# nghorbani/moshpp

Hardware: NVIDIA H100
Metric: mocap frames solved/sec (Stage-II) (higher is better)
Workload: dtype f32

## Files before the change

moshpp_b200/csrc/mosh2.cu:

```cuda
#include "../../include/mosh2.h"

#include <cuda_runtime.h>

#include <cstdarg>
#include <cstdio>
#include <cstdlib>
#include <algorithm>
#include <cstring>
#include <map>
#include <mutex>
#include <new>
#include <string>
#include <vector>

#include "mesh_distance.cuh"
#include "mosh2_device.cuh"
#include "mosh2_host.h"

namespace {

thread_local std::string g_err;

int fail(int code, const char *fmt, ...) {
    char buf[512];
// ... 270 lines not shown
    int *d_status = nullptr, *d_counters = nullptr, *d_totals = nullptr;
    long long *d_prof = nullptr;
    void *h_obs = nullptr, *h_out = nullptr;
    uint8_t *h_vis = nullptr;
    void *d_lin = nullptr;
    size_t lin_bytes = 0;
    int lin_mode = 0, lin_step = 1;
    mosh2_host::LinLayout lin{};
    struct RangeSlot { void *h = nullptr, *d = nullptr; size_t bytes = 0; cudaEvent_t done = nullptr; };
    std::vector<RangeSlot> range_slots;
    int *h_status = nullptr, *h_counters = nullptr;
    std::vector<mosh2_model *> models;
    std::vector<unsigned char> h_models;
    void *d_models = nullptr;
    int *d_model_of_chunk = nullptr;
    size_t n_obs = 0, n_out = 0;
    size_t o_fullpose = 0, o_pose = 0, o_trans = 0, o_dmpls = 0, o_mk = 0, o_errs = 0;
};

namespace {

template <class real, bool BIG>
cudaError_t launch_kernel(mosh2_job *j, const mosh2::Model<real> &m, const mosh2::Job<real> &job, int threads) {
    const mosh2_host::Layout<real, BIG> L = mosh2_host::layout<real, BIG>(m, mosh2::kSmemHeader, threads);
    const cudaError_t e = cudaFuncSetAttribute(mosh2_stageii_kernel<real, BIG>, cudaFuncAttributeMaxDynamicSharedMemorySize, int(j->smem));
    if (e != cudaSuccess) return e;
    mosh2_stageii_kernel<real, BIG><<<j->launch_blocks, threads, j->smem, j->stream>>>(m, job, L.w, L.d);
    return cudaGetLastError();
}

template <class real, bool BIG>
cudaError_t launch_multi_kernel(mosh2_job *j, const mosh2::Job<real> &job, int threads) {
    const mosh2::Model<real> &m = *reinterpret_cast<const mosh2::Model<real> *>(j->h_models.data());
    const mosh2_host::Layout<real, BIG> L = mosh2_host::layout<real, BIG>(m, mosh2_host::multi_smem_header<real>(), threads);
    const cudaError_t e = cudaFuncSetAttribute(mosh2_stageii_multi_kernel<real, BIG>, cudaFuncAttributeMaxDynamicSharedMemorySize, int(j->smem));
    if (e != cudaSuccess) return e;
    mosh2_stageii_multi_kernel<real, BIG><<<j->launch_blocks, threads, j->smem, j->stream>>>(
        static_cast<const mosh2::Model<real> *>(j->d_models), j->d_model_of_chunk, job, L.w, L.d);
    return cudaGetLastError();
}

template <class real>
int launch(mosh2_job *j, const mosh2::Model<real> &m) {
    mosh2::Job<real> job{};
    job.n_frames = j->n_frames; job.n_chunks = j->n_chunks;
    job.chunk_tab = j->d_chunk_tab; job.chunk_ids = j->subset ? j->d_chunk_ids : nullptr;
    job.warm_x = static_cast<real *>(j->d_warm_x); job.warm_f = j->d_warm_f; job.merge_tol = j->merge_tol;
    job.obs = static_cast<const real *>(j->d_obs);
    job.vis = j->d_vis;
    real *out = static_cast<real *>(j->d_out);
    job.fullpose = out + j->o_fullpose; job.pose = out + j->o_pose; job.trans = out + j->o_trans;
    job.dmpls = j->model->n_dmpl ? out + j->o_dmpls : nullptr;
    job.markers_sim = out + j->o_mk; job.errs = out + j->o_errs;
    job.status = j->d_status; job.counters = j->d_counters; job.totals = j->d_totals; job.prof = j->d_prof;
    job.gws = static_cast<char *>(j->d_gws); job.gws_stride = j->gws_stride;
    job.lin_mode = j->lin_mode; job.lin_step = j->lin_step;
    if (j->lin_mode) mosh2_host::bind_lin(job, static_cast<real *>(j->d_lin), j->lin);
// ... 197 lines not shown
template <class real>
int make_multi(mosh2_job *j, mosh2_model *const *models, int32_t n_models, int32_t n_seq, const int32_t *frame_counts,
               const int32_t *model_of_seq) {
    auto dev_model = [](mosh2_model *mm) -> mosh2::Model<real> & {
        if constexpr (sizeof(real) == 8) return mm->f64.m; else return mm->f32.m;
    };
    mosh2::Model<real> plan = dev_model(models[0]);
    size_t smem = 0, gws = 0;
    int big = 0;
    plan_workspace(plan, &smem, &gws, &big, mosh2_host::multi_smem_header<real>());
    if (smem > kMaxSmem) return fail(MOSH2_E_TOO_LARGE, "model needs %zu bytes of shared memory per block (max %zu)", smem, kMaxSmem);
    const int dv = j->model->device;
    const size_t stride = big ? gws : 0;
    if (stride > j->gws_stride) {
        g_blocks.put(dv, j->d_gws);
        j->d_gws = nullptr;
        CU(g_blocks.get(dv, stride * j->n_chunks, &j->d_gws));
    }
    j->smem = smem; j->big_in_global = big; j->gws_stride = stride;
    std::vector<mosh2::Model<real>> recs(n_models);
    for (int k = 0; k < n_models; ++k) {
        recs[k] = dev_model(models[k]);
        recs[k].tile_markers = plan.tile_markers;
        recs[k].dev_no_tc = plan.dev_no_tc;
    }
    j->h_models.assign(reinterpret_cast<const unsigned char *>(recs.data()), reinterpret_cast<const unsigned char *>(recs.data() + n_models));
    const std::vector<int> moc = mosh2_host::model_of_chunks(j->tab0, frame_counts, n_seq, model_of_seq);
    CU(g_blocks.get(dv, j->h_models.size(), &j->d_models));
    CU(g_blocks.get(dv, moc.size() * sizeof(int), reinterpret_cast<void **>(&j->d_model_of_chunk)));
    CU(cudaMemcpy(j->d_models, j->h_models.data(), j->h_models.size(), cudaMemcpyHostToDevice));
    CU(cudaMemcpy(j->d_model_of_chunk, moc.data(), moc.size() * sizeof(int), cudaMemcpyHostToDevice));
    j->models.assign(models, models + n_models);
    return 0;
}

}

extern "C" {

int mosh2_job_create_multi(mosh2_model *const *models, int32_t n_models, const mosh2_options *opt, int32_t n_seq,
                           const int32_t *frame_counts, const int32_t *model_of_seq, const mosh2_schedule *sched,
                           int32_t precision, mosh2_job **out) {
    if (!models || n_models < 1 || !opt || !out || n_seq < 1 || !frame_counts || !model_of_seq) return fail(MOSH2_E_INVALID, "bad argument");
    if (precision != MOSH2_F32 && precision != MOSH2_F64) return fail(MOSH2_E_INVALID, "precision must be MOSH2_F32 or MOSH2_F64");
    *out = nullptr;
    for (int k = 0; k < n_models; ++k) {
        if (!models[k]) return fail(MOSH2_E_INVALID, "model %d is NULL", k);
// ... 430 lines not shown
```

moshpp_b200/csrc/mosh2_device.cuh:

```cuda
#pragma once
#include <math.h>
#include <stdint.h>

#if defined(__CUDACC__) && !defined(MOSH2_EMU)
#define M2_HD __host__ __device__ __forceinline__
#define M2_D __device__ __forceinline__
#define M2_NOINLINE __device__ __noinline__
#define M2_SYNC() __syncthreads()
#define M2_WSYNC() __syncwarp()
#define M2_GPU 1
#else
#define M2_HD inline
#define M2_D inline
#define M2_NOINLINE static inline
#define M2_SYNC() ((void)0)
#define M2_WSYNC() ((void)0)
#define M2_GPU 0
#endif

#if defined(MOSH2_PROFILE) && M2_GPU
#define M2_T0() long long t_prev_ = clock64()
#define M2_TACC(slot) do { if (cta.tid == 0) { const long long t_now_ = clock64(); w.prof[(slot) + prof_base] += t_now_ - t_prev_; t_prev_ = t_now_; } } while (0)
#define M2_TRESET() do { t_prev_ = clock64(); } while (0)
#else
// ... 307 lines not shown
    return v;
}

template <class real, bool BIG = false>
struct Work {
    SPtr<real> x, xt, pose_prev, velo_tgt, dm_tgt;
    SPtr<real> fullpose, Rl, dRl, Jp, Rg, tg, vp, pj, Rsk, mk, rm, obs, py, pq, pxg;
    BPtr<real, BIG> Loc, MtR, u, dtg;
    SPtr<real> Linv, Pn, g, Ag, dgn, d, tmp, ds;
    BPtr<real, BIG> Jt, Jf, A, Lm;
    SPtr<real> red, sc, hct;
    SPtr<int> colmap, colsrc, jlist, isc;
    SPtr<int> st_colmap, st_colsrc, st_jlist, st_meta;
    SPtr<int> c_parents, c_fk_order, c_wj, c_free1, c_free2, c_pids;
    SPtr<int> c_tin, c_tsz;
    SPtr<real> c_wv, c_v0, c_coefs, c_j0, c_hmean, c_pmeans, c_pnlw;
    SPtr<real> c_jd;
    SPtr<long long> prof;
    SPtr<uint8_t> vis;
    SPtr<uint32_t> c_chain;
    SPtr<uint8_t> c_amask;
    SPtr<unsigned long long> mbar;
    uint32_t stage_ofs, stage_bytes;
    int tc_ok;
    int tc;
};

constexpr int kMaxDepth = 16;
constexpr int kDR = 28;
constexpr int kM3 = 12;
#if M2_GPU
namespace tc {
__device__ __forceinline__ uint32_t smem_u32(const void *p) { return static_cast<uint32_t>(__cvta_generic_to_shared(p)); }
__device__ __forceinline__ uint32_t to_tf32(float v) { uint32_t r; asm("cvt.rna.tf32.f32 %0, %1;" : "=r"(r) : "f"(v)); return r; }
__device__ __forceinline__ void mma_tf32_m16n8k8(float (&d)[4], const uint32_t (&a)[4], uint32_t b0, uint32_t b1) {
    asm volatile("mma.sync.aligned.m16n8k8.row.col.f32.tf32.tf32.f32 {%0, %1, %2, %3}, {%4, %5, %6, %7}, {%8, %9}, {%0, %1, %2, %3};"
                 : "+f"(d[0]), "+f"(d[1]), "+f"(d[2]), "+f"(d[3]) : "r"(a[0]), "r"(a[1]), "r"(a[2]), "r"(a[3]), "r"(b0), "r"(b1));
}
__device__ __forceinline__ void jtj_block_tf32(const float *J, int ld, int rows, int cols, int i0, int j0,
                                               float (&hh)[2][4], float (&cr)[2][4]) {
    const int lane = threadIdx.x & 31, g = lane >> 2, t = lane & 3;
    const int ca0 = i0 + g, ca1 = i0 + 8 + g, cb0 = j0 + g, cb1 = j0 + 8 + g;
    for (int k0 = 0; k0 < rows; k0 += 8) {
        const int k1 = k0 + t, k2 = k0 + t + 4;
        const float *r1 = J + (k1 < rows ? k1 : 0) * ld, *r2 = J + (k2 < rows ? k2 : 0) * ld;
        const bool in1 = k1 < rows, in2 = k2 < rows;
        const float av[4] = {(in1 && ca0 < cols) ? r1[ca0] : 0.f, (in1 && ca1 < cols) ? r1[ca1] : 0.f,
                             (in2 && ca0 < cols) ? r2[ca0] : 0.f, (in2 && ca1 < cols) ? r2[ca1] : 0.f};
// ... 58 lines not shown
struct Arena {
    size_t off;
    template <class T> M2_HD uint32_t take(size_t n) {
        off = (off + 15) & ~size_t(15);
        const size_t o = off;
        off += n * sizeof(T);
        return uint32_t(o);
    }
};

template <class real, bool BIG>
M2_HD void carve(Work<real, BIG> &w, const Dims &d, const Model<real> &m, Arena &S, Arena &G) {
    const int hct_size = m.hct_size;
    Arena &B = BIG ? G : S;
    w.x.ofs = S.take<real>(d.NX); w.xt.ofs = S.take<real>(d.NX);
    w.pose_prev.ofs = S.take<real>(d.PR); w.velo_tgt.ofs = S.take<real>(d.PR); w.dm_tgt.ofs = S.take<real>(d.nd + 1);
    w.fullpose.ofs = S.take<real>(d.PF); w.Rl.ofs = S.take<real>(9 * d.nJ); w.dRl.ofs = S.take<real>(kDR * d.nJ);
    w.Jp.ofs = S.take<real>(3 * d.nJ); w.Rg.ofs = S.take<real>(9 * d.nJ); w.tg.ofs = S.take<real>(3 * d.nJ);
    w.vp.ofs = S.take<real>(3 * d.S); w.pj.ofs = S.take<real>(3 * d.S * d.kw); w.Rsk.ofs = S.take<real>(9 * d.S);
    w.mk.ofs = S.take<real>(3 * d.M); w.rm.ofs = S.take<real>(3 * d.M); w.obs.ofs = S.take<real>(3 * d.M);
    w.py.ofs = S.take<real>(d.K * d.D + 1); w.pq.ofs = S.take<real>(d.K + 1); w.pxg.ofs = S.take<real>(d.D + 1);
    {
        w.A.ofs = B.take<real>(size_t(d.n2) * d.lda);
        w.tc_ok = (sizeof(real) == 4 && !BIG && !m.dev_no_tc) ? 1 : 0;
        w.tc = 0;
        const size_t mark_b = B.off;
        w.Lm.ofs = B.take<real>(size_t(d.n2 + 1) * d.ld);
        const size_t end_b = B.off;
        B.off = mark_b;
        w.Jt.ofs = B.take<real>(d.jt_size);
        w.Jf.ofs = B.take<real>(3 * d.tmk * d.npad);
        w.Loc.ofs = B.take<real>(3 * kM3 * d.M); w.MtR.ofs = B.take<real>(kM3 * d.S);
        w.u.ofs = B.take<real>(kM3 * d.nJ); w.dtg.ofs = B.take<real>(3 * d.nJ * d.nd + 1);
        if (B.off < end_b) B.off = end_b;
    }
    w.Linv.ofs = S.take<real>(size_t((d.n2 + kCholNB - 1) / kCholNB) * kCholNB * kCholNB);
    w.Pn.ofs = S.take<real>(size_t(kCholNB) * d.ldp);
    w.g.ofs = S.take<real>(d.npad); w.Ag.ofs = S.take<real>(d.npad); w.dgn.ofs = S.take<real>(d.npad);
    w.d.ofs = S.take<real>(d.npad); w.tmp.ofs = S.take<real>(d.npad); w.ds.ofs = S.take<real>(d.npad);
    w.red.ofs = S.take<real>(8 * 33); w.sc.ofs = S.take<real>(16);
    w.colmap.ofs = S.take<int>(d.NX); w.colsrc.ofs = S.take<int>(d.n2); w.jlist.ofs = S.take<int>(d.nJ); w.isc.ofs = S.take<int>(8);
    w.st_colmap.ofs = S.take<int>(2 * d.NX); w.st_colsrc.ofs = S.take<int>(2 * d.n2); w.st_jlist.ofs = S.take<int>(2 * d.nJ); w.st_meta.ofs = S.take<int>(4);
    w.prof.ofs = S.take<long long>(32);
    w.mbar.ofs = S.take<unsigned long long>(1);
    w.vis.ofs = S.take<uint8_t>(d.M);
    S.off = (S.off + 15) & ~size_t(15);
    w.stage_ofs = uint32_t(S.off);
    w.c_parents.ofs = S.take<int>(d.nJ); w.c_fk_order.ofs = S.take<int>(d.nJ);
    w.c_wj.ofs = S.take<int>(d.S * d.kw); w.c_free1.ofs = S.take<int>(d.n1); w.c_free2.ofs = S.take<int>(d.n2);
    w.c_pids.ofs = S.take<int>(d.D + 1);
    w.c_wv.ofs = S.take<real>(d.S * d.kw); w.c_v0.ofs = S.take<real>(3 * d.S); w.c_coefs.ofs = S.take<real>(3 * d.M);
    w.c_j0.ofs = S.take<real>(3 * d.nJ); w.c_hmean.ofs = S.take<real>(m.n_hand_full + 1);
    w.c_pmeans.ofs = S.take<real>(d.K * d.D + 1); w.c_pnlw.ofs = S.take<real>(d.K + 1);
    w.hct.ofs = S.take<real>(hct_size + 4);
    if (!BIG) w.c_jd.ofs = S.take<real>(size_t(3) * d.nJ * d.nd + 1);
    S.off = (S.off + 15) & ~size_t(15);
// ... 30 lines not shown
    const Job<real> &job;
    const Work<real, BIG> &w;
    const Cta cta;
    const Dims &d;
    real wd, wp_frame, wH, wv, wdm, wex, wF, wxp;
    int nvis, njl;
    bool has_velo, has_extrap, hand_free;
    int n_iter, n_eval, n_build, n_min, frame_flags;
    int prof_base = 0;
    bool fwd_at_x = false;
    bool fwd_has_prior = false;
    bool resuming = false;
    int root_turns = 0;
    real resume_diff = 0;
    int lin_f = -1;

    M2_D Solver(const Model<real> &m_, const Job<real> &j_, const Work<real, BIG> &w_, const Dims &d_, Cta c_)
        : m(m_), job(j_), w(w_), cta(c_), d(d_) {}

#define CTA_FOR(i, n) _Pragma("unroll 1") for (int i = cta.tid; i < (n); i += cta.nthr)

    M2_D const real *jdir() const { return BIG ? m.jd : static_cast<const real *>(w.c_jd); }

    M2_D void cta_max(real *v) {
#if M2_GPU
        real x = v[0];
#pragma unroll
        for (int o = 16; o > 0; o >>= 1) { const real y = __shfl_xor_sync(0xffffffffu, x, o); x = y > x ? y : x; }
        const int lane = cta.tid & 31, warp = cta.tid >> 5, nwarp = (cta.nthr + 31) >> 5;
        if (lane == 0) w.red[warp] = x;
        __syncthreads();
        if (cta.tid == 0) { real mx = w.red[0]; for (int q = 1; q < nwarp; ++q) mx = w.red[q] > mx ? w.red[q] : mx; w.red[32] = mx; }
        __syncthreads();
        v[0] = w.red[32];
        __syncthreads();
#else
        (void)v;
#endif
    }

    M2_D void fk(int l, int nl) {
        for (int j = l; j < d.nJ; j += nl) {
            uint32_t cw[kMaxDepth / 4];
#pragma unroll
            for (int q = 0; q < kMaxDepth / 4; ++q) cw[q] = w.c_chain[j * (kMaxDepth / 4) + q];
            int prev = int(cw[0] & 255u);
// ... 44 lines not shown
            for (int j = j0; j < j1; j += 2) {
                const bool two = j + 1 < j1;
                const real *P = m.pdc + (size_t(j - 1) * 27 + c) * cs + 4 * sq, *Q = P + (two ? 27 * cs : 0);
                Vec4<real> pa[9], pb[9];
#pragma unroll
                for (int e = 0; e < 9; ++e) pa[e] = ld4(P + 3 * e * cs);
#pragma unroll
                for (int e = 0; e < 9; ++e) pb[e] = ld4(Q + 3 * e * cs);
                const real *R = w.Rl + 9 * j, *R2 = R + (two ? 9 : 0);
                const real tw = two ? real(1) : real(0);
#pragma unroll
                for (int e = 0; e < 9; ++e) {
                    const real id = (e == 0 || e == 4 || e == 8) ? real(1) : real(0);
                    const real fa = R[e] - id, fb = (R2[e] - id) * tw;
                    acc[0] += pa[e].x * fa + pb[e].x * fb;
                    acc[1] += pa[e].y * fa + pb[e].y * fb;
                    acc[2] += pa[e].z * fa + pb[e].z * fb;
                    acc[3] += pa[e].w * fa + pb[e].w * fb;
                }
            }
#pragma unroll
            for (int q = 0; q < 4; ++q) {
                const int sl = 4 * sq + q;
                if (sl < d.S) w.Jt[(g * d.S + sl) * 3 + c] = acc[q];
            }
        }
    }

    M2_D void eval(const real *xs, const StepCfg<real> &c, bool reuse = false) {
        ++n_eval;
        M2_T0();
        const real *th = xs + 3;
        const real *dl = xs + 3 + d.PR;
        if (!reuse) {
        CTA_FOR(i, d.PF) {
            real v;
            if (i < m.body_dof) {
                v = th[i];
            } else {
                const int q = i - m.body_dof;
                v = w.c_hmean[q];
                for (int b = 0; b < m.hb_n; ++b) {
                    const HandBlock hb = m.hb[b];
                    if (q >= hb.q0 && q < hb.q1) {
                        const real *ct = w.hct + hb.ct_off + (q - hb.q0) * hb.rw4;
                        for (int r = hb.r0; r < hb.r1; ++r) v += th[m.body_dof + r] * ct[r - hb.r0];
                    }
// ... 90 lines not shown
        }
#if defined(MOSH2_PROFILE) && M2_GPU
        __syncthreads();
        M2_TACC(19);
#endif
        CTA_FOR(s, d.S) {
            real vpo[3];
#pragma unroll
            for (int q = 0; q < 3; ++q) vpo[q] = w.c_v0[3 * s + q];
            for (int e0 = 0; e0 < d.nd; e0 += 8) {
                real sv[24];
#pragma unroll
                for (int u = 0; u < 24; ++u) {
                    const int q = u >> 3, e = e0 + (u & 7);
                    sv[u] = e < d.nd ? m.sd[(3 * s + q) * d.nd + e] : real(0);
                }
#pragma unroll
                for (int u = 0; u < 24; ++u) {
                    const int e = e0 + (u & 7);
                    vpo[u >> 3] += sv[u] * (e < d.nd ? dl[e] : real(0));
                }
            }
            for (int q = 0; q < 3; ++q)
                for (int g = 0; g < nbg; ++g) vpo[q] += w.Jt[(g * d.S + s) * 3 + q];
            real v[3] = {0, 0, 0};
            real Rs[9] = {0, 0, 0, 0, 0, 0, 0, 0, 0};
            for (int i = 0; i < d.kw; ++i) {
                const int j = w.c_wj[s * d.kw + i];
                real *pp = w.pj + 3 * (s * d.kw + i);
                if (j < 0) { pp[0] = pp[1] = pp[2] = 0; continue; }
                const real wt = w.c_wv[s * d.kw + i];
                real dv[3] = {vpo[0] - w.Jp[3 * j], vpo[1] - w.Jp[3 * j + 1], vpo[2] - w.Jp[3 * j + 2]};
                real o[3];
                mat3_vec(w.Rg + 9 * j, dv, o);
                for (int q = 0; q < 3; ++q) {
                    pp[q] = o[q] + w.tg[3 * j + q];
                    v[q] += wt * pp[q];
                }
                for (int q = 0; q < 9; ++q) Rs[q] += wt * w.Rg[9 * j + q];
            }
            for (int q = 0; q < 3; ++q) w.vp[3 * s + q] = v[q] + xs[q];
            for (int q = 0; q < 9; ++q) w.Rsk[9 * s + q] = Rs[q];
        }
        M2_SYNC();
        M2_TACC(3);
        }
        if (reuse) {
// ... 224 lines not shown
#pragma unroll
            for (int u = 0; u < kMaxDepth / 4; ++u) cw[u] = w.c_chain[j * (kMaxDepth / 4) + u];
            int prev = int(cw[0] & 255u);
            real acc[3];
            for (int r = 0; r < 3; ++r) acc[r] = jdir()[(3 * prev + r) * d.nd + i];
            for (int k = 1; k < kMaxDepth; ++k) {
                const int cj = int((cw[k >> 2] >> (8 * (k & 3))) & 255u);
                if (cj == 255) break;
                real dj[3], t[3];
                for (int r = 0; r < 3; ++r) dj[r] = jdir()[(3 * cj + r) * d.nd + i] - jdir()[(3 * prev + r) * d.nd + i];
                mat3_vec(w.Rg + 9 * prev, dj, t);
                for (int r = 0; r < 3; ++r) acc[r] = acc[r] + t[r];
                prev = cj;
            }
            real *o = w.dtg + 3 * (j * d.nd + i);
            for (int r = 0; r < 3; ++r) o[r] = acc[r];
        }
    }

    M2_D void tile_pose_columns(int t0, int tm) {
#if M2_GPU
        const int lane = cta.tid & 31, warp = cta.tid >> 5, nwarp = cta.nthr >> 5;
        const int t = lane % 3, grp = lane / 3;
        const int nmg = (tm + 9) / 10, nch = nwarp / nmg;
        const int mg = warp % nmg, ch = warp / nmg;
        const int ml = mg * 10 + grp;
        const bool valid = lane < 30 && ml < tm;
        if (ch < nch) {
            const int mi = t0 + (valid ? ml : 0), sl = 3 * mi + t;
            const real sc = (valid && w.vis[mi]) ? wd : real(0);
            real Mt[9], Lc[9];
            slot_mats(sl, Mt, Lc);
            const real *Pslot = m.pd4 + size_t(sl) * 4;
            const int src1 = lane - t + (t + 2) % 3, src2 = lane - t + (t + 1) % 3;
#pragma unroll 1
            for (int ji = ch; ji < njl; ji += nch) {
                const int a = w.jlist[ji];
                real blk[9];
                slot_pose_block(sl, a, Mt, Lc, Pslot, blk);
                real col3[3];
#pragma unroll
                for (int r = 0; r < 3; ++r) {
                    const real b0 = blk[3 * r], b1 = blk[3 * r + 1], b2 = blk[3 * r + 2];
                    const real own = sel3(t, b0, b1, b2);
                    const real to1 = sel3(t, b1, b2, b0);
                    const real to2 = sel3(t, b2, b0, b1);
                    col3[r] = own + __shfl_sync(0xffffffffu, to1, src1) + __shfl_sync(0xffffffffu, to2, src2);
                }
                if (valid) pose_col_store(ml, a, t, sc, col3[0], col3[1], col3[2]);
            }
        }
#else
        for (int gi = 0; gi < tm * njl; ++gi) {
            const int ml = gi % tm, a = w.jlist[gi / tm], mi = t0 + ml;
            real blk[9] = {0, 0, 0, 0, 0, 0, 0, 0, 0};
            for (int t = 0; t < 3; ++t) {
                const int sl = 3 * mi + t;
                real Mt[9], Lc[9], part[9];
                slot_mats(sl, Mt, Lc);
                slot_pose_block(sl, a, Mt, Lc, m.pd4 + size_t(sl) * 4, part);
                for (int q = 0; q < 9; ++q) blk[q] += part[q];
            }
            const real sc = w.vis[mi] ? wd : real(0);
            for (int k = 0; k < 3; ++k) pose_col_store(ml, a, k, sc, blk[k], blk[3 + k], blk[6 + k]);
        }
#endif
    }

    M2_D void tile_linear_columns(int t0, int tm) {
        CTA_FOR(it, tm * d.nd) {
            const int ml = it / d.nd, i = it - ml * d.nd, mi = t0 + ml;
            real val[3] = {0, 0, 0};
            real sdv[9];
// ... 82 lines not shown
#pragma unroll
            for (int ni = 0; ni < 2; ++ni)
#pragma unroll
                for (int e = 0; e < 2; ++e) {
                    const int i = i0 + 8 * mi + g, j = j0 + 8 * ni + 2 * tq + e;
                    old[mi][ni][e] = (j < n && i <= j) ? w.A[i * ld + j] : real(0);
                }
#pragma unroll
        for (int mi = 0; mi < 2; ++mi)
#pragma unroll
            for (int ni = 0; ni < 2; ++ni)
#pragma unroll
                for (int e = 0; e < 2; ++e) {
                    const int i = i0 + 8 * mi + g, j = j0 + 8 * ni + 2 * tq + e;
                    if (j < n && i <= j) {
                        const real v = old[mi][ni][e] + c[mi][ni][e];
                        w.A[i * ld + j] = v;
                        if (i < j) w.A[j * ld + i] = v;
                    }
                }
    }
#endif

    M2_D void tile_normal_equations(int t0, int tm, int n) {
        const int trows = 3 * tm, ld = d.lda;
        if (lin_f >= 0 && job.lin_J) {
            real *Jo = job.lin_J + (size_t(lin_f) * 3 * d.M + 3 * t0) * n;
            CTA_FOR(idx, trows * n) { const int row = idx / n, cc = idx - row * n; Jo[idx] = w.Jf[row * d.npad + cc]; }
        }
#if M2_GPU
        if constexpr (sizeof(real) == 8) {
            const int lane = cta.tid & 31, warp = cta.tid >> 5, nwarp = cta.nthr >> 5;
            const int g = lane >> 2, tq = lane & 3;
            const int nb16 = (n + 15) >> 4, ntile = nb16 * (nb16 + 1) / 2;
            for (int tile = warp; tile < ntile; tile += nwarp) {
                int ti, tj;
                upper_block(tile, nb16, ti, tj);
                const int i0 = 16 * ti, j0 = 16 * tj;
                double c[2][2][2] = {{{0, 0}, {0, 0}}, {{0, 0}, {0, 0}}};
                const int ca0 = i0 + g, ca1 = i0 + 8 + g, cb0 = j0 + g, cb1 = j0 + 8 + g;
                for (int k0 = 0; k0 < trows; k0 += 4) {
                    const int k = k0 + tq;
                    const bool kin = k < trows;
                    const real *Jr = w.Jf + (kin ? k : 0) * d.npad;
                    const double a0 = (kin && ca0 < d.npad) ? double(Jr[ca0]) : 0.0, a1 = (kin && ca1 < d.npad) ? double(Jr[ca1]) : 0.0;
                    const double b0 = (kin && cb0 < d.npad) ? double(Jr[cb0]) : 0.0, b1 = (kin && cb1 < d.npad) ? double(Jr[cb1]) : 0.0;
                    dmma_m8n8k4(c[0][0][0], c[0][0][1], a0, b0);
                    dmma_m8n8k4(c[0][1][0], c[0][1][1], a0, b1);
                    dmma_m8n8k4(c[1][0][0], c[1][0][1], a1, b0);
                    dmma_m8n8k4(c[1][1][0], c[1][1][1], a1, b1);
                }
                add_upper_block16(i0, j0, n, c);
            }
        } else if (w.tc) {
            const int warp = cta.tid >> 5, nwarp = cta.nthr >> 5;
            const int nb16 = (n + 15) >> 4, ntile = nb16 * (nb16 + 1) / 2;
            for (int tile = warp; tile < ntile; tile += nwarp) {
                int ti, tj;
                upper_block(tile, nb16, ti, tj);
                const int i0 = 16 * ti, j0 = 16 * tj;
                float hh[2][4] = {{0, 0, 0, 0}, {0, 0, 0, 0}}, cr[2][4] = {{0, 0, 0, 0}, {0, 0, 0, 0}};
                tc::jtj_block_tf32(w.Jf, d.npad, trows, d.npad, i0, j0, hh, cr);
                real c[2][2][2];
#pragma unroll
                for (int mi = 0; mi < 2; ++mi)
#pragma unroll
                    for (int ni = 0; ni < 2; ++ni)
#pragma unroll
                        for (int e = 0; e < 2; ++e) c[mi][ni][e] = hh[ni][2 * mi + e] + cr[ni][2 * mi + e];
                add_upper_block16(i0, j0, n, c);
            }
        } else
#endif
        {
            const int nb = (n + kBS - 1) / kBS, nblk = nb * (nb + 1) / 2;
            CTA_FOR(b, nblk) {
                int bi, bj;
                upper_block(b, nb, bi, bj);
                real acc[kBS * kBS];
#pragma unroll
                for (int q = 0; q < kBS * kBS; ++q) acc[q] = 0;
                for (int row = 0; row < trows; row += 4) {
                    Vec4<real> av[4], bv[4];
#pragma unroll
                    for (int u = 0; u < 4; ++u) {
                        const real *Jr = w.Jf + (row + u < trows ? row + u : trows - 1) * d.npad;
                        av[u] = ld4(Jr + bi * kBS);
                        bv[u] = ld4(Jr + bj * kBS);
                    }
#pragma unroll
                    for (int u = 0; u < 4; ++u)
                        if (row + u < trows) {
                            const real ai[4] = {av[u].x, av[u].y, av[u].z, av[u].w}, bjv[4] = {bv[u].x, bv[u].y, bv[u].z, bv[u].w};
#pragma unroll
                            for (int p = 0; p < kBS; ++p)
#pragma unroll
                                for (int q = 0; q < kBS; ++q) acc[p * kBS + q] += ai[p] * bjv[q];
                        }
                }
#pragma unroll
                for (int p = 0; p < kBS; ++p)
#pragma unroll
                    for (int q = 0; q < kBS; ++q) {
                        const int i = bi * kBS + p, j = bj * kBS + q;
                        if (j < n && i <= j) {
                            w.A[i * ld + j] += acc[p * kBS + q];
                            if (i < j) w.A[j * ld + i] += acc[p * kBS + q];
                        }
                    }
            }
        }
        int jr_tid = cta.tid;
#if M2_GPU
        if (sizeof(real) == 8 || w.tc) {
            const int nb16 = (n + 15) >> 4, nwarp = cta.nthr >> 5;
            jr_tid = (cta.tid + cta.nthr - 32 * ((nb16 * (nb16 + 1) / 2) % nwarp)) % cta.nthr;
        }
#endif
#pragma unroll 1
        for (int cc = jr_tid; cc < n; cc += cta.nthr) {
            real s = 0;
            for (int row = 0; row < trows; row += 6) {
                real jv[6];
#pragma unroll
                for (int u = 0; u < 6; ++u) jv[u] = w.Jf[(row + u < trows ? row + u : trows - 1) * d.npad + cc];
#pragma unroll
                for (int u = 0; u < 6; ++u) if (row + u < trows) s += jv[u] * w.rm[3 * t0 + row + u];
            }
            w.g[cc] -= s;
        }
    }

    M2_D void closed_form_terms(const real *xs, const StepCfg<real> &c) {
        const real *th = xs + 3;
        const real *dl = xs + 3 + d.PR;
        const int n = c.n, ld = d.lda;
        if (c.wp > real(0)) {
            const int D = d.D, ks = w.isc[0];
            const real w2 = c.wp * c.wp;
// ... 57 lines not shown
            w.A[cc * ld + cc] += da;
            w.g[cc] -= dg;
        }
        if (c.wp > real(0) && m.n_jang) {
            M2_SYNC();
            CTA_FOR(i, m.n_jang) {
                const int ci = w.colmap[3 + m.jang_id[i]];
                if (ci >= 0) {
                    const real sg = m.jang_sign[i], ex = r_exp(real(2) * sg * th[m.jang_id[i]]);
                    const real Jd = real(4) * c.wp * sg * ex, rr = real(2) * c.wp * ex;
                    w.A[ci * ld + ci] += Jd * Jd;
                    w.g[ci] -= Jd * rr;
                }
            }
        }
    }

    M2_D void build(const real *xs, const StepCfg<real> &c) {
        ++n_build;
        M2_T0();
        const int n = c.n;
        joint_axes();
        CTA_FOR(mi, d.M) marker_local_jacobian(mi);
        CTA_FOR(i, n * d.lda) w.A[i] = 0;
        CTA_FOR(i, n) w.g[i] = 0;
        dtg_chains();
        M2_SYNC();
        CTA_FOR(s, d.S) mat3_mul(w.Loc + kM3 * s, w.Rsk + 9 * s, w.MtR + kM3 * s);
        M2_SYNC();
        M2_TACC(6);
        for (int t0 = 0; t0 < d.M; t0 += d.tmk) {
            const int tm = (d.M - t0 < d.tmk) ? d.M - t0 : d.tmk;
            tile_pose_columns(t0, tm);
            tile_linear_columns(t0, tm);
            tile_translation_columns(t0, tm, n);
            M2_SYNC();
            M2_TACC(7);
            tile_hand_columns(t0, tm);
            M2_SYNC();
            M2_TACC(8);
            tile_normal_equations(t0, tm, n);
            M2_SYNC();
            M2_TACC(9);
        }
        closed_form_terms(xs, c);
        M2_SYNC();
        M2_TACC(10);
// ... 955 lines not shown
```

moshpp_b200/csrc/mosh2_host.h:

```cpp
#pragma once
#include <algorithm>
#include <cstdarg>
#include <cstddef>
#include <cstdio>
#include <cstdlib>
#include <string>
#include <type_traits>
#include <vector>

#include "../../include/mosh2.h"
#include "mosh2_device.cuh"

namespace mosh2_host {

inline int reject(std::string *msg, int code, const char *fmt, ...) {
    char buf[512];
    va_list ap;
    va_start(ap, fmt);
    vsnprintf(buf, sizeof buf, fmt, ap);
    va_end(ap);
    *msg = buf;
    return code;
}

// ... 69 lines not shown
    mosh2::Model<real> m{};
    m.nJ = d.n_joints; m.M = d.n_markers; m.body_dof = d.body_dof; m.p_red = d.p_red;
    m.n_hand_red = d.n_hand_red; m.n_hand_full = d.n_hand_full; m.nd = d.n_dmpl; m.kw = d.kw;
    m.prior_k = d.prior_k; m.prior_d = d.prior_d; m.prior_d4 = (d.prior_d + 3) & ~3;
    m.n1 = d.n_free1; m.n2 = d.n_free2; m.finger_lo = d.finger_lo; m.finger_hi = d.finger_hi;
    m.n_expr = d.n_expr; m.face_lo = d.face_lo; m.face_hi = d.face_hi;
    m.n_jang = d.n_jangles;
    for (int i = 0; i < d.n_jangles && i < mosh2::kMaxJangles; ++i) { m.jang_id[i] = d.jangles_ids[i]; m.jang_sign[i] = real(d.jangles_signs[i]); }
    mosh2::HandBlock blocks[mosh2::kMaxHandBlocks];
    m.hb_n = hand_blocks(d.hand_comps, d.n_hand_red, d.n_hand_full, blocks, *hct);
    for (int b = 0; b < m.hb_n; ++b) m.hb[b] = blocks[b];
    m.hct_size = int(hct->size());
    return m;
}

template <class real, bool BIG>
struct Layout {
    mosh2::Dims d;
    mosh2::Work<real, BIG> w;
    size_t smem, gws;
};

template <class real, bool BIG>
Layout<real, BIG> layout(const mosh2::Model<real> &m, unsigned header = mosh2::kSmemHeader, int threads = 1) {
    Layout<real, BIG> L{};
    L.d = mosh2::make_dims(m);
    mosh2::Arena S{header}, G{0};
    mosh2::carve<real, BIG>(L.w, L.d, m, S, G);
    L.w.tc = (L.w.tc_ok && threads >= 128) ? 1 : 0;
    L.smem = S.off;
    L.gws = G.off;
    return L;
}

template <class real, class Place>
bool build_model(const mosh2_model_desc &d, mosh2::Model<real> &m, Place &&place) {
    std::vector<double> hct;
    m = model_dims<real>(d, &hct);
    const size_t nJ = d.n_joints, S = size_t(3) * d.n_markers, nd = d.n_dmpl, K = d.prior_k, D = d.prior_d, D4 = m.prior_d4;
    std::vector<int> order(nJ), depth(nJ, 0), ids(D);
    for (size_t j = 0; j < nJ; ++j) { int dj = 0; for (int a = d.parents[j]; a >= 0; a = d.parents[a]) ++dj; depth[j] = dj; }
    for (size_t j = 0; j < nJ; ++j) order[j] = int(j);
    std::stable_sort(order.begin(), order.end(), [&](int a, int b) { return depth[a] < depth[b]; });
    for (size_t i = 0; i < D; ++i) ids[i] = d.prior_ids ? d.prior_ids[i] : d.prior_off + int(i);
    const size_t Sp = (S + 3) & ~size_t(3);
    std::vector<double> pdc((nJ - 1) * 27 * Sp, 0.0), pd4((nJ - 1) * 9 * S * 4, 0.0);
    for (size_t j = 0; j + 1 < nJ; ++j)
        for (size_t sl = 0; sl < S; ++sl)
            for (int c = 0; c < 3; ++c)
                for (int e = 0; e < 9; ++e) {
                    const double v = d.pd[(j * 3 * S + 3 * sl + c) * 9 + e];
                    pdc[((j * 9 + e) * 3 + c) * Sp + sl] = v;
// ... 59 lines not shown
            const int rec[mosh2::kChunkRec] = {s0 + f, s0 + int(e), s0, warmup, warm_full, 0};
            tab.insert(tab.end(), rec, rec + mosh2::kChunkRec);
            f = int(e);
        }
        s0 += F;
    }
    return tab;
}

inline std::vector<int> schedule_table(const mosh2_schedule *s, const int *frame_counts, int n_seq) {
    const int chunk_len = s && s->chunk_len > 0 ? s->chunk_len : 0, warmup = s && s->chunk_warmup > 0 ? s->chunk_warmup : 0;
    const int warm_full = (!s || s->warmup_full < 0 || s->warmup_full > warmup) ? warmup : s->warmup_full;
    const int first_extra = (s && s->first_extra > 0 && chunk_len > 0 && warmup > 0) ? s->first_extra : 0;
    return chunk_table(frame_counts, n_seq, chunk_len, warmup, warm_full, first_extra);
}

template <class real>
constexpr unsigned multi_smem_header() { return mosh2::kSmemHeader + ((unsigned(sizeof(mosh2::Model<real>)) + 15u) & ~15u); }

constexpr size_t kMaxSmem = 227 * 1024;

template <class real>
void plan_workspace(mosh2::Model<real> &m, size_t *smem, size_t *gws, int *big, unsigned header = mosh2::kSmemHeader) {
    const int tries[3][2] = {{20, 0}, {10, 0}, {10, 1}};
    const char *dev_tile = getenv("MOSH2_DEV_TILE");
    const bool dev_big = getenv("MOSH2_DEV_BIG") != nullptr;
    for (int pass = dev_big ? 2 : ((dev_tile && atoi(dev_tile) == 10) ? 1 : 0); pass < 3; ++pass) {
        m.tile_markers = tries[pass][0];
        m.dev_no_tc = getenv("MOSH2_DEV_NO_TC") ? 1 : 0;
        *big = tries[pass][1];
        size_t s, g;
        if (*big) { const Layout<real, true> L = layout<real, true>(m, header); s = L.smem; g = L.gws; }
        else { const Layout<real, false> L = layout<real, false>(m, header); s = L.smem; g = L.gws; }
        *smem = (s + 15) & ~size_t(15);
        *gws = (g + 255) & ~size_t(255);
        if (s <= kMaxSmem) return;
    }
}

inline std::vector<int> model_of_chunks(const std::vector<int> &tab, const int *frame_counts, int n_seq, const int *model_of_seq) {
    std::vector<int> out(tab.size() / mosh2::kChunkRec);
    int q = 0, s0 = 0;
    for (size_t c = 0; c < out.size(); ++c) {
        const int first = tab[c * mosh2::kChunkRec + 2];
        while (q + 1 < n_seq && s0 + frame_counts[q] <= first) s0 += frame_counts[q++];
        out[c] = model_of_seq[q];
    }
    return out;
}

template <class real>
const char *kernel_shape_mismatch(const mosh2::Model<real> &a, const mosh2::Model<real> &b) {
    const struct { const char *name; int a, b; } f[] = {
// ... 55 lines not shown
```

Measured before the change: 117,200.

## Add single-pass marker tiling and rebalanced register-tiled JtJ, drop TF32 path

The planner now first tries a marker tile large enough to cover all markers in f32, so the normal equations are built in one pass. In that mode A is written directly instead of zeroed and accumulated, and the Jacobian scratch overlaps the A region. The TF32 tensor-core JtJ path is removed and replaced by a 4x8 register-tiled scalar JtJ whose row range is split across lanes and reduced with warp shuffles to balance work. Pose column computation is also chunked by warp capacity. This adds shared-memory pressure from bigger tiles and gives up tensor cores in exchange for fewer passes and less A read-modify-write.

```diff
diff --git a/moshpp_b200/csrc/mosh2.cu b/moshpp_b200/csrc/mosh2.cu
--- a/moshpp_b200/csrc/mosh2.cu
+++ b/moshpp_b200/csrc/mosh2.cu
@@ -316,7 +316,7 @@
 
 template <class real, bool BIG>
 cudaError_t launch_kernel(mosh2_job *j, const mosh2::Model<real> &m, const mosh2::Job<real> &job, int threads) {
-    const mosh2_host::Layout<real, BIG> L = mosh2_host::layout<real, BIG>(m, mosh2::kSmemHeader, threads);
+    const mosh2_host::Layout<real, BIG> L = mosh2_host::layout<real, BIG>(m, mosh2::kSmemHeader);
     const cudaError_t e = cudaFuncSetAttribute(mosh2_stageii_kernel<real, BIG>, cudaFuncAttributeMaxDynamicSharedMemorySize, int(j->smem));
     if (e != cudaSuccess) return e;
     mosh2_stageii_kernel<real, BIG><<<j->launch_blocks, threads, j->smem, j->stream>>>(m, job, L.w, L.d);
@@ -326,7 +326,7 @@
 template <class real, bool BIG>
 cudaError_t launch_multi_kernel(mosh2_job *j, const mosh2::Job<real> &job, int threads) {
     const mosh2::Model<real> &m = *reinterpret_cast<const mosh2::Model<real> *>(j->h_models.data());
-    const mosh2_host::Layout<real, BIG> L = mosh2_host::layout<real, BIG>(m, mosh2_host::multi_smem_header<real>(), threads);
+    const mosh2_host::Layout<real, BIG> L = mosh2_host::layout<real, BIG>(m, mosh2_host::multi_smem_header<real>());
     const cudaError_t e = cudaFuncSetAttribute(mosh2_stageii_multi_kernel<real, BIG>, cudaFuncAttributeMaxDynamicSharedMemorySize, int(j->smem));
     if (e != cudaSuccess) return e;
     mosh2_stageii_multi_kernel<real, BIG><<<j->launch_blocks, threads, j->smem, j->stream>>>(
@@ -570,7 +570,6 @@
     for (int k = 0; k < n_models; ++k) {
         recs[k] = dev_model(models[k]);
         recs[k].tile_markers = plan.tile_markers;
-        recs[k].dev_no_tc = plan.dev_no_tc;
     }
     j->h_models.assign(reinterpret_cast<const unsigned char *>(recs.data()), reinterpret_cast<const unsigned char *>(recs.data() + n_models));
     const std::vector<int> moc = mosh2_host::model_of_chunks(j->tab0, frame_counts, n_seq, model_of_seq);
diff --git a/moshpp_b200/csrc/mosh2_device.cuh b/moshpp_b200/csrc/mosh2_device.cuh
--- a/moshpp_b200/csrc/mosh2_device.cuh
+++ b/moshpp_b200/csrc/mosh2_device.cuh
@@ -353,8 +353,8 @@
     SPtr<uint8_t> c_amask;
     SPtr<unsigned long long> mbar;
     uint32_t stage_ofs, stage_bytes;
-    int tc_ok;
-    int tc;
+    BPtr<real, BIG> Pb;
+    int one_pass;
 };
 
 constexpr int kMaxDepth = 16;
@@ -459,16 +459,29 @@
     w.py.ofs = S.take<real>(d.K * d.D + 1); w.pq.ofs = S.take<real>(d.K + 1); w.pxg.ofs = S.take<real>(d.D + 1);
     {
         w.A.ofs = B.take<real>(size_t(d.n2) * d.lda);
-        w.tc_ok = (sizeof(real) == 4 && !BIG && !m.dev_no_tc) ? 1 : 0;
-        w.tc = 0;
+        w.one_pass = (sizeof(real) == 4 && !BIG && d.tmk >= d.M) ? 1 : 0;
         const size_t mark_b = B.off;
         w.Lm.ofs = B.take<real>(size_t(d.n2 + 1) * d.ld);
         const size_t end_b = B.off;
-        B.off = mark_b;
-        w.Jt.ofs = B.take<real>(d.jt_size);
-        w.Jf.ofs = B.take<real>(3 * d.tmk * d.npad);
-        w.Loc.ofs = B.take<real>(3 * kM3 * d.M); w.MtR.ofs = B.take<real>(kM3 * d.S);
-        w.u.ofs = B.take<real>(kM3 * d.nJ); w.dtg.ofs = B.take<real>(3 * d.nJ * d.nd + 1);
+        auto scratch = [&] {
+            w.Loc.ofs = B.take<real>(3 * kM3 * d.M); w.MtR.ofs = B.take<real>(kM3 * d.S);
+            w.u.ofs = B.take<real>(kM3 * d.nJ); w.dtg.ofs = B.take<real>(3 * d.nJ * d.nd + 1);
+        };
+        if (w.one_pass) {
+            B.off = w.A.ofs;
+            w.Jt.ofs = B.take<real>(3 * d.tmk * d.NCt);
+            scratch();
+            if (B.off < mark_b) B.off = mark_b;
+            const int jf = 3 * d.tmk * d.npad, pb = kBlendGroups * 9 * d.M + 16;
+            w.Jf.ofs = B.take<real>(jf > pb ? jf : pb);
+            w.Pb.ofs = w.Jf.ofs;
+        } else {
+            B.off = mark_b;
+            w.Jt.ofs = B.take<real>(d.jt_size);
+            w.Jf.ofs = B.take<real>(3 * d.tmk * d.npad);
+            scratch();
+            w.Pb.ofs = w.Jt.ofs;
+        }
         if (B.off < end_b) B.off = end_b;
     }
     w.Linv.ofs = S.take<real>(size_t((d.n2 + kCholNB - 1) / kCholNB) * kCholNB * kCholNB);
@@ -545,6 +558,8 @@
 
     M2_D const real *jdir() const { return BIG ? m.jd : static_cast<const real *>(w.c_jd); }
 
+    M2_D bool one_pass() const { return sizeof(real) == 4 && !BIG && w.one_pass; }
+
     M2_D void cta_max(real *v) {
 #if M2_GPU
         real x = v[0];
@@ -635,7 +650,7 @@
 #pragma unroll
             for (int q = 0; q < 4; ++q) {
                 const int sl = 4 * sq + q;
-                if (sl < d.S) w.Jt[(g * d.S + sl) * 3 + c] = acc[q];
+                if (sl < d.S) w.Pb[(g * d.S + sl) * 3 + c] = acc[q];
             }
         }
     }
@@ -772,7 +787,7 @@
                 }
             }
             for (int q = 0; q < 3; ++q)
-                for (int g = 0; g < nbg; ++g) vpo[q] += w.Jt[(g * d.S + s) * 3 + q];
+                for (int g = 0; g < nbg; ++g) vpo[q] += w.Pb[(g * d.S + s) * 3 + q];
             real v[3] = {0, 0, 0};
             real Rs[9] = {0, 0, 0, 0, 0, 0, 0, 0, 0};
             for (int i = 0; i < d.kw; ++i) {
@@ -1043,33 +1058,41 @@
 #if M2_GPU
         const int lane = cta.tid & 31, warp = cta.tid >> 5, nwarp = cta.nthr >> 5;
         const int t = lane % 3, grp = lane / 3;
-        const int nmg = (tm + 9) / 10, nch = nwarp / nmg;
-        const int mg = warp % nmg, ch = warp / nmg;
-        const int ml = mg * 10 + grp;
-        const bool valid = lane < 30 && ml < tm;
-        if (ch < nch) {
-            const int mi = t0 + (valid ? ml : 0), sl = 3 * mi + t;
-            const real sc = (valid && w.vis[mi]) ? wd : real(0);
-            real Mt[9], Lc[9];
-            slot_mats(sl, Mt, Lc);
-            const real *Pslot = m.pd4 + size_t(sl) * 4;
-            const int src1 = lane - t + (t + 2) % 3, src2 = lane - t + (t + 1) % 3;
+        auto part = [&](int p0, int pm) {
+            const int nmg = (pm + 9) / 10, nch = nwarp / nmg;
+            const int mg = warp % nmg, ch = warp / nmg;
+            const int ml = p0 + mg * 10 + grp;
+            const bool valid = lane < 30 && ml < p0 + pm;
+            if (ch < nch) {
+                const int mi = t0 + (valid ? ml : 0), sl = 3 * mi + t;
+                const real sc = (valid && w.vis[mi]) ? wd : real(0);
+                real Mt[9], Lc[9];
+                slot_mats(sl, Mt, Lc);
+                const real *Pslot = m.pd4 + size_t(sl) * 4;
+                const int src1 = lane - t + (t + 2) % 3, src2 = lane - t + (t + 1) % 3;
 #pragma unroll 1
-            for (int ji = ch; ji < njl; ji += nch) {
-                const int a = w.jlist[ji];
-                real blk[9];
-                slot_pose_block(sl, a, Mt, Lc, Pslot, blk);
-                real col3[3];
-#pragma unroll
-                for (int r = 0; r < 3; ++r) {
-                    const real b0 = blk[3 * r], b1 = blk[3 * r + 1], b2 = blk[3 * r + 2];
-                    const real own = sel3(t, b0, b1, b2);
-                    const real to1 = sel3(t, b1, b2, b0);
-                    const real to2 = sel3(t, b2, b0, b1);
-                    col3[r] = own + __shfl_sync(0xffffffffu, to1, src1) + __shfl_sync(0xffffffffu, to2, src2);
-                }
-                if (valid) pose_col_store(ml, a, t, sc, col3[0], col3[1], col3[2]);
-            }
+                for (int ji = ch; ji < njl; ji += nch) {
+                    const int a = w.jlist[ji];
+                    real blk[9];
+                    slot_pose_block(sl, a, Mt, Lc, Pslot, blk);
+                    real col3[3];
+#pragma unroll
+                    for (int r = 0; r < 3; ++r) {
+                        const real b0 = blk[3 * r], b1 = blk[3 * r + 1], b2 = blk[3 * r + 2];
+                        const real own = sel3(t, b0, b1, b2);
+                        const real to1 = sel3(t, b1, b2, b0);
+                        const real to2 = sel3(t, b2, b0, b1);
+                        col3[r] = own + __shfl_sync(0xffffffffu, to1, src1) + __shfl_sync(0xffffffffu, to2, src2);
+                    }
+                    if (valid) pose_col_store(ml, a, t, sc, col3[0], col3[1], col3[2]);
+                }
+            }
+        };
+        if constexpr (sizeof(real) == 4) {
+#pragma unroll 1
+            for (int p0 = 0; p0 < tm; p0 += 10 * nwarp) part(p0, tm - p0 < 10 * nwarp ? tm - p0 : 10 * nwarp);
+        } else {
+            part(0, tm);
         }
 #else
         for (int gi = 0; gi < tm * njl; ++gi) {
@@ -1198,12 +1221,33 @@
     }
 #endif
 
+    template <int R>
+    M2_D void jtj_rows(const real *Jr, int i0, int j0, int j4, real (&acc)[32]) const {
+        Vec4<real> av[R], bv[R], cv[R];
+#pragma unroll
+        for (int u = 0; u < R; ++u) {
+            av[u] = ld4(Jr + u * d.npad + i0);
+            bv[u] = ld4(Jr + u * d.npad + j0);
+            cv[u] = ld4(Jr + u * d.npad + j4);
+        }
+#pragma unroll
+        for (int u = 0; u < R; ++u) {
+            const real ai[4] = {av[u].x, av[u].y, av[u].z, av[u].w};
+            const real bj8[8] = {bv[u].x, bv[u].y, bv[u].z, bv[u].w, cv[u].x, cv[u].y, cv[u].z, cv[u].w};
+#pragma unroll
+            for (int p = 0; p < 4; ++p)
+#pragma unroll
+                for (int q = 0; q < 8; ++q) acc[8 * p + q] += ai[p] * bj8[q];
+        }
+    }
+
     M2_D void tile_normal_equations(int t0, int tm, int n) {
         const int trows = 3 * tm, ld = d.lda;
         if (lin_f >= 0 && job.lin_J) {
             real *Jo = job.lin_J + (size_t(lin_f) * 3 * d.M + 3 * t0) * n;
             CTA_FOR(idx, trows * n) { const int row = idx / n, cc = idx - row * n; Jo[idx] = w.Jf[row * d.npad + cc]; }
         }
+        int jr_skip = 0;
 #if M2_GPU
         if constexpr (sizeof(real) == 8) {
             const int lane = cta.tid & 31, warp = cta.tid >> 5, nwarp = cta.nthr >> 5;
@@ -1228,69 +1272,63 @@
                 }
                 add_upper_block16(i0, j0, n, c);
             }
-        } else if (w.tc) {
-            const int warp = cta.tid >> 5, nwarp = cta.nthr >> 5;
-            const int nb16 = (n + 15) >> 4, ntile = nb16 * (nb16 + 1) / 2;
-            for (int tile = warp; tile < ntile; tile += nwarp) {
-                int ti, tj;
-                upper_block(tile, nb16, ti, tj);
-                const int i0 = 16 * ti, j0 = 16 * tj;
-                float hh[2][4] = {{0, 0, 0, 0}, {0, 0, 0, 0}}, cr[2][4] = {{0, 0, 0, 0}, {0, 0, 0, 0}};
-                tc::jtj_block_tf32(w.Jf, d.npad, trows, d.npad, i0, j0, hh, cr);
-                real c[2][2][2];
-#pragma unroll
-                for (int mi = 0; mi < 2; ++mi)
-#pragma unroll
-                    for (int ni = 0; ni < 2; ++ni)
-#pragma unroll
-                        for (int e = 0; e < 2; ++e) c[mi][ni][e] = hh[ni][2 * mi + e] + cr[ni][2 * mi + e];
-                add_upper_block16(i0, j0, n, c);
-            }
         } else
 #endif
         {
-            const int nb = (n + kBS - 1) / kBS, nblk = nb * (nb + 1) / 2;
-            CTA_FOR(b, nblk) {
-                int bi, bj;
-                upper_block(b, nb, bi, bj);
-                real acc[kBS * kBS];
-#pragma unroll
-                for (int q = 0; q < kBS * kBS; ++q) acc[q] = 0;
-                for (int row = 0; row < trows; row += 4) {
-                    Vec4<real> av[4], bv[4];
-#pragma unroll
-                    for (int u = 0; u < 4; ++u) {
-                        const real *Jr = w.Jf + (row + u < trows ? row + u : trows - 1) * d.npad;
-                        av[u] = ld4(Jr + bi * kBS);
-                        bv[u] = ld4(Jr + bj * kBS);
-                    }
-#pragma unroll
-                    for (int u = 0; u < 4; ++u)
-                        if (row + u < trows) {
-                            const real ai[4] = {av[u].x, av[u].y, av[u].z, av[u].w}, bjv[4] = {bv[u].x, bv[u].y, bv[u].z, bv[u].w};
-#pragma unroll
-                            for (int p = 0; p < kBS; ++p)
-#pragma unroll
-                                for (int q = 0; q < kBS; ++q) acc[p * kBS + q] += ai[p] * bjv[q];
+            const int nbi = (n + 3) >> 2, nbj = (n + 7) >> 3;
+            auto col_tiles = [nbi](int bj) { return 2 * bj + 2 < nbi ? 2 * bj + 2 : nbi; };
+            int ntile = 0;
+            for (int bj = 0; bj < nbj; ++bj) ntile += col_tiles(bj);
+            int S = 1;
+#if M2_GPU
+            while (S < 4 && 2 * S * ntile <= cta.nthr) S *= 2;
+#endif
+            const int per = 32 / S, nitem = S == 1 ? ntile : (ntile + per - 1) / per * 32;
+            CTA_FOR(it, nitem) {
+                const int lane = it & 31, part = S == 1 ? 0 : lane / per, tile = S == 1 ? it : (it >> 5) * per + lane % per;
+                int bi = tile < ntile ? tile : 0, bj = 0;
+                while (bi >= col_tiles(bj)) { bi -= col_tiles(bj); ++bj; }
+                const int i0 = 4 * bi, j0 = 8 * bj;
+                const int j4 = j0 + 4 < d.npad ? j0 + 4 : j0;
+                real acc[32];
+#pragma unroll
+                for (int q = 0; q < 32; ++q) acc[q] = 0;
+                constexpr int U = BIG ? 2 : 4;
+                const int r0 = part * trows / S, r1 = (part + 1) * trows / S, full = r1 - (r1 - r0) % U;
+                const real *Jr = w.Jf + r0 * d.npad;
+#pragma unroll 1
+                for (int row = r0; row < full; row += U, Jr += U * d.npad) jtj_rows<U>(Jr, i0, j0, j4, acc);
+#pragma unroll 1
+                for (int row = full; row < r1; ++row, Jr += d.npad) jtj_rows<1>(Jr, i0, j0, j4, acc);
+#if M2_GPU
+                for (int o = 16; o >= per; o >>= 1)
+#pragma unroll
+                    for (int q = 0; q < 32; ++q) acc[q] += __shfl_xor_sync(0xffffffffu, acc[q], o);
+#endif
+                if (part == 0 && tile < ntile) {
+#pragma unroll
+                    for (int p = 0; p < 4; ++p)
+#pragma unroll
+                        for (int q = 0; q < 8; ++q) {
+                            const int i = i0 + p, j = j0 + q;
+                            if (i <= j && j < n) {
+                                const real v = one_pass() ? acc[8 * p + q] : w.A[i * ld + j] + acc[8 * p + q];
+                                w.A[i * ld + j] = v;
+                                if (i < j) w.A[j * ld + i] = v;
+                            }
                         }
                 }
-#pragma unroll
-                for (int p = 0; p < kBS; ++p)
-#pragma unroll
-                    for (int q = 0; q < kBS; ++q) {
-                        const int i = bi * kBS + p, j = bj * kBS + q;
-                        if (j < n && i <= j) {
-                            w.A[i * ld + j] += acc[p * kBS + q];
-                            if (i < j) w.A[j * ld + i] += acc[p * kBS + q];
-                        }
-                    }
-            }
+            }
+            const int extra = nitem % cta.nthr;
+            jr_skip = (extra + 31) & ~31;
         }
         int jr_tid = cta.tid;
 #if M2_GPU
-        if (sizeof(real) == 8 || w.tc) {
+        if constexpr (sizeof(real) == 8) {
             const int nb16 = (n + 15) >> 4, nwarp = cta.nthr >> 5;
             jr_tid = (cta.tid + cta.nthr - 32 * ((nb16 * (nb16 + 1) / 2) % nwarp)) % cta.nthr;
+        } else {
+            jr_tid = (cta.tid + cta.nthr - jr_skip) % cta.nthr;
         }
 #endif
 #pragma unroll 1
@@ -1394,7 +1432,7 @@
         const int n = c.n;
         joint_axes();
         CTA_FOR(mi, d.M) marker_local_jacobian(mi);
-        CTA_FOR(i, n * d.lda) w.A[i] = 0;
+        if (!one_pass()) CTA_FOR(i, n * d.lda) w.A[i] = 0;
         CTA_FOR(i, n) w.g[i] = 0;
         dtg_chains();
         M2_SYNC();
diff --git a/moshpp_b200/csrc/mosh2_host.h b/moshpp_b200/csrc/mosh2_host.h
--- a/moshpp_b200/csrc/mosh2_host.h
+++ b/moshpp_b200/csrc/mosh2_host.h
@@ -115,12 +115,11 @@
 };
 
 template <class real, bool BIG>
-Layout<real, BIG> layout(const mosh2::Model<real> &m, unsigned header = mosh2::kSmemHeader, int threads = 1) {
+Layout<real, BIG> layout(const mosh2::Model<real> &m, unsigned header = mosh2::kSmemHeader) {
     Layout<real, BIG> L{};
     L.d = mosh2::make_dims(m);
     mosh2::Arena S{header}, G{0};
     mosh2::carve<real, BIG>(L.w, L.d, m, S, G);
-    L.w.tc = (L.w.tc_ok && threads >= 128) ? 1 : 0;
     L.smem = S.off;
     L.gws = G.off;
     return L;
@@ -226,13 +225,19 @@
 
 template <class real>
 void plan_workspace(mosh2::Model<real> &m, size_t *smem, size_t *gws, int *big, unsigned header = mosh2::kSmemHeader) {
-    const int tries[3][2] = {{20, 0}, {10, 0}, {10, 1}};
+    std::vector<std::pair<int, int>> tries;
     const char *dev_tile = getenv("MOSH2_DEV_TILE");
     const bool dev_big = getenv("MOSH2_DEV_BIG") != nullptr;
-    for (int pass = dev_big ? 2 : ((dev_tile && atoi(dev_tile) == 10) ? 1 : 0); pass < 3; ++pass) {
-        m.tile_markers = tries[pass][0];
-        m.dev_no_tc = getenv("MOSH2_DEV_NO_TC") ? 1 : 0;
-        *big = tries[pass][1];
+    if (!dev_big && !(dev_tile && atoi(dev_tile) == 10)) {
+        if (sizeof(real) == 4)
+            for (int k = 1; (m.M + k - 1) / k > 20; ++k) tries.push_back({(m.M + k - 1) / k, 0});
+        tries.push_back({20, 0});
+    }
+    if (!dev_big) tries.push_back({10, 0});
+    tries.push_back({10, 1});
+    for (const auto &t : tries) {
+        m.tile_markers = t.first;
+        *big = t.second;
         size_t s, g;
         if (*big) { const Layout<real, true> L = layout<real, true>(m, header); s = L.smem; g = L.gws; }
         else { const Layout<real, false> L = layout<real, false>(m, header); s = L.smem; g = L.gws; }
```

Result: faster. 131,200, median of 6 (+11.9%).
